# snimu/mixture-of-tokenizers

Hardware: NVIDIA B200
Metric: byte-mix embedding fwd+bwd tokens/sec (higher is better)
Workload: dtype bf16

## Files before the change

mixture-of-tokenizers_b200/csrc/mot_embed.cu:

```cuda
#include <algorithm>

#include "mot_embed_bwd_sum.cuh"

namespace mot {

__global__ void plan_hist_kernel(const int32_t* tok, long long N, int V, int* cnt) {
  pdl_launch_dependents();
  pdl_wait();
  for (long long i = (long long)blockIdx.x * blockDim.x + threadIdx.x; i < N; i += (long long)gridDim.x * blockDim.x)
    atomicAdd(&cnt[clampi(ld_g(tok + i), V - 1)], 1);
}

constexpr int kScanTile = 1024;
__global__ void __launch_bounds__(256) plan_scan_kernel(EmbedParams p) {
  __shared__ int wsum[8];
  __shared__ int wcarry[8];
  const int tid = threadIdx.x, lane = tid & 31, warp = tid >> 5;
  const int base = blockIdx.x * kScanTile;
  pdl_launch_dependents();
  pdl_wait();
  int carry = 0;
  for (int v = tid * 4; v < base; v += 256 * 4) {
    const int4 c = *reinterpret_cast<const int4*>(p.cnt + v);
    carry += c.x + c.y + c.z + c.w;
// ... 114 lines not shown
  }
  if (d->row_stride != 0 || d->col_offset != 0) {
    const long long ld = d->row_stride ? d->row_stride : d->out_dim;
    if (d->col_offset < 0 || ld < (long long)d->col_offset + d->out_dim || ld > 0x7fffffffLL) return MOT_ERR_BAD_ARG;
    if (ld % 8 || d->col_offset % 8) return MOT_ERR_MISALIGNED;
  }
  if (d->dp_slabs < 0 || d->dp_slabs > 64) return MOT_ERR_BAD_ARG;
  if ((d->flags & MOT_F_TTB_PULL_LEFT) && (d->flags & MOT_F_TTB_PULL_RIGHT)) return MOT_ERR_BAD_ARG;
  if ((d->flags & MOT_F_TTB_NEXT_TOK) && !(d->flags & MOT_F_TTB_PULL_RIGHT)) return MOT_ERR_BAD_ARG;
  if ((d->flags & MOT_F_IDS_FROM_TTB) && has_bytes) {
    if (d->ttb_dtype < MOT_TTB_I16 || d->ttb_dtype > MOT_TTB_BF16) return MOT_ERR_UNSUPPORTED;
    if (d->flags & (MOT_F_TTB_SCRAMBLE | MOT_F_TTB_PULL_LEFT | MOT_F_TTB_PULL_RIGHT))
      if (d->seq_len <= 0 || d->n_tokens % d->seq_len) return MOT_ERR_BAD_ARG;
    if (d->flags & (MOT_F_TTB_PULL_LEFT | MOT_F_TTB_PULL_RIGHT)) {
      if (d->tok_vocab <= 0) return MOT_ERR_BAD_ARG;
      if (d->pad_id != (int16_t)d->pad_id || d->eot_id != (int16_t)d->eot_id) return MOT_ERR_BAD_ARG;
    }
  }
  return MOT_OK;
}

static int validate(const MotDesc* d) {
  if (int rc = validate_desc(d)) return rc;
  if ((d->flags & MOT_F_BYTE_NORM) && d->combine != MOT_TOK_ONLY && d->byte_dim > 256) return MOT_ERR_UNSUPPORTED;
  constexpr int kMaxCols = 8 * 32 * 8;
  if (d->combine == MOT_CONCAT && !(d->flags & (MOT_F_OUT_NORM | MOT_F_HAS_LAMBDAS))) {
    if (d->tok_dim > kMaxCols || (long long)d->bpt * d->byte_dim > kMaxCols) return MOT_ERR_UNSUPPORTED;
  } else if (d->out_dim > kMaxCols) {
    return MOT_ERR_UNSUPPORTED;
  }
  return MOT_OK;
}

static bool aligned16(const void* p) { return (reinterpret_cast<uintptr_t>(p) & 15u) == 0; }

static void fill_params(const MotDesc* d, EmbedParams& p) {
  p = EmbedParams{};
  p.N = d->n_tokens;
  p.T = d->seq_len > 0 ? d->seq_len : (d->n_tokens > 0 ? d->n_tokens : 1);
  p.V = d->tok_vocab;
  p.Vb = d->combine == MOT_TOK_ONLY ? 0 : d->byte_vocab;
  p.bpt = d->combine == MOT_TOK_ONLY ? 0 : d->bpt;
  p.Dt = d->combine == MOT_BYTES_ONLY ? 0 : d->tok_dim;
  p.bd = d->combine == MOT_TOK_ONLY ? 8 : d->byte_dim;
  p.Do = d->out_dim;
  p.combine = d->combine;
  p.flags = d->flags;
  p.ttb_dtype = d->ttb_dtype;
  p.pad_eot = (d->pad_id & 0xffff) | (d->eot_id << 16);
  p.n_chunks = d->out_dim / kChunk;
  p.io_ld = d->row_stride ? d->row_stride : d->out_dim;
  p.io_col = d->col_offset;
  p.eps = d->eps;
  p.R = stream_chunk(d->n_tokens, kBwdThreads / 32);
  p.n_rep = kByteRep;
  p.stages = 4;
  p.tab_smem = 1;
  p.v_lo = 0;
  p.v_hi = p.V;
  p.last_slab = 1;
}

static bool concat_splits(const MotDesc* d) {
  return d->combine == MOT_CONCAT && !(d->flags & (MOT_F_OUT_NORM | MOT_F_HAS_LAMBDAS));
}
static void split_params(const MotDesc* d, EmbedParams& pt, EmbedParams& pb) {
  const int db = d->bpt * d->byte_dim;
  const bool bytes_first = (d->flags & MOT_F_BYTES_FIRST) != 0;
  MotDesc dt = *d, dbd = *d;
  dt.combine = MOT_TOK_ONLY;
  dt.out_dim = d->tok_dim;
  dt.flags = d->flags & MOT_F_TOK_NORM;
  dbd.combine = MOT_BYTES_ONLY;
  dbd.out_dim = db;
  dbd.flags = d->flags & ~(MOT_F_TOK_NORM | MOT_F_BYTES_FIRST);
  fill_params(&dt, pt);
  fill_params(&dbd, pb);
  pt.io_ld = pb.io_ld = d->row_stride ? d->row_stride : d->out_dim;
  pt.io_col = d->col_offset + (bytes_first ? db : 0);
  pb.io_col = d->col_offset + (bytes_first ? 0 : d->tok_dim);
}

struct WsLayout {
  size_t cnt, byte_acc, lam_acc, partial, zero_end, off, order, stok, total;
};

static WsLayout ws_layout(const EmbedParams& p, int dp_slabs = 0) {
  WsLayout w{};
  const long long V = p.V > 0 ? p.V : 1, N = p.N > 0 ? p.N : 1;
  int r_min = std::min(p.R, stream_chunk(N, kSumThreads / 32));
  if (dp_slabs > 1) r_min = std::min(r_min, stream_chunk_slab(N, dp_slabs, kSumThreads / 32));
  const long long n_stream_chunks = (N + r_min - 1) / r_min;
  size_t o = 0;
  auto take = [&](size_t bytes) {
    size_t at = o;
    o = align_up(o + bytes, 256);
    return at;
  };
  w.cnt = take((size_t)V * 4);
  w.byte_acc = take((size_t)p.n_rep * (p.Vb > 0 ? p.Vb : 1) * p.bd * 4);
  w.lam_acc = take(16);
  w.partial = take((size_t)n_stream_chunks * (p.Dt > 0 ? p.Dt : 8) * 4);
  w.zero_end = o;
  w.off = take((size_t)(V + 1) * 4);
  w.order = take((size_t)N * 4);
  w.stok = take((size_t)N * 4);
  w.total = o;
  return w;
}

static void bind_ws(EmbedParams& p, const WsLayout& w, void* ws) {
  char* b = reinterpret_cast<char*>(ws);
  p.cnt = reinterpret_cast<int*>(b + w.cnt);
  p.byte_acc = reinterpret_cast<float*>(b + w.byte_acc);
  p.lam_acc = reinterpret_cast<float*>(b + w.lam_acc);
  p.off = reinterpret_cast<int*>(b + w.off);
  p.order = reinterpret_cast<int*>(b + w.order);
  p.stok = reinterpret_cast<int*>(b + w.stok);
  p.partial = reinterpret_cast<float*>(b + w.partial);
  p.chk = chk_record();
  p.n_slots = (int)((w.zero_end - w.partial) / ((size_t)(p.Dt > 0 ? p.Dt : 8) * 4));
}

static int run_plan(const EmbedParams& p, cudaStream_t s) {
  if (p.combine == MOT_BYTES_ONLY || p.N == 0) return MOT_OK;
  long long hb = (p.N + 255) / 256;
  if (hb > 2048) hb = 2048;
  launch_pdl(plan_hist_kernel, dim3((unsigned)hb), dim3(256), 0, s, p.tok, p.N, p.V, p.cnt);
  launch_pdl(plan_scan_kernel, dim3((unsigned)((p.V + kScanTile - 1) / kScanTile)), dim3(256), 0, s, p);
  launch_pdl(plan_fill_kernel, dim3((unsigned)((p.N + 255) / 256)), dim3(256), 0, s, p);
  count_launch(3);
  return check_launch();
}

}

using namespace mot;

extern "C" size_t mot_embed_workspace_bytes(const MotDesc* d) {
  if (validate(d) != MOT_OK) return 0;
  EmbedParams p;
  fill_params(d, p);
  return ws_layout(p, d->dp_slabs).total;
}

extern "C" int mot_embed_fwd(const MotDesc* d, const int32_t* tok, const void* byte_ids, const void* ttb,
                             const void* E_tok, const void* E_byte, const float* lam, void* out, void* stream) {
  return mot_embed_fwd_ex(d, tok, byte_ids, ttb, E_tok, E_byte, lam, nullptr, out, nullptr, stream);
}

extern "C" int mot_embed_fwd_ex(const MotDesc* d, const int32_t* tok, const void* byte_ids, const void* ttb,
                                const void* E_tok, const void* E_byte, const float* lam, const void* addend, void* out,
                                float* rstd_out, void* stream) {
  if (int rc = validate(d)) return rc;
  if (addend && (concat_splits(d) || d->row_stride != 0 || d->col_offset != 0)) return MOT_ERR_UNSUPPORTED;
  if (!aligned16(addend)) return MOT_ERR_MISALIGNED;
  if (d->n_tokens == 0) return MOT_OK;
  const bool has_tok = d->combine != MOT_BYTES_ONLY, has_bytes = d->combine != MOT_TOK_ONLY;
  if (!out || (has_tok && (!tok || !E_tok)) || (has_bytes && !E_byte)) return MOT_ERR_BAD_ARG;
  if (has_bytes) {
    if (d->flags & MOT_F_IDS_FROM_TTB) { if (!ttb || !tok) return MOT_ERR_BAD_ARG; }
    else if (!byte_ids) return MOT_ERR_BAD_ARG;
  }
  if ((d->flags & MOT_F_HAS_LAMBDAS) && !lam) return MOT_ERR_BAD_ARG;
  if (!aligned16(out) || !aligned16(E_tok) || !aligned16(E_byte)) return MOT_ERR_MISALIGNED;
  cudaStream_t s = reinterpret_cast<cudaStream_t>(stream);
  if (concat_splits(d)) {
    EmbedParams pt, pb;
    split_params(d, pt, pb);
    for (EmbedParams* q : {&pt, &pb}) {
      q->tok = tok; q->ids = byte_ids; q->ttb = ttb; q->E_tok = E_tok; q->E_byte = E_byte; q->lam = lam; q->out = out;
      if (int rc = d->dtype == MOT_BF16 ? dispatch_fwd_bf16(*q, s) : dispatch_fwd_f32(*q, s)) return rc;
    }
    return MOT_OK;
  }
  EmbedParams p;
  fill_params(d, p);
  p.tok = tok; p.ids = byte_ids; p.ttb = ttb; p.E_tok = E_tok; p.E_byte = E_byte; p.lam = lam; p.out = out;
  p.rstd_out = (d->flags & MOT_F_OUT_NORM) ? rstd_out : nullptr;
  p.addend = addend;
  if (addend) return d->dtype == MOT_BF16 ? dispatch_fwd_addend_bf16(p, s) : dispatch_fwd_addend_f32(p, s);
  return d->dtype == MOT_BF16 ? dispatch_fwd_bf16(p, s) : dispatch_fwd_f32(p, s);
}

extern "C" int mot_embed_workspace_init(const MotDesc* d, void* workspace, size_t ws_bytes, void* stream) {
  if (int rc = validate(d)) return rc;
  if (!workspace) return MOT_ERR_BAD_ARG;
  EmbedParams p;
  fill_params(d, p);
  const WsLayout w = ws_layout(p, d->dp_slabs);
  if (ws_bytes < w.total) return MOT_ERR_WORKSPACE;
  if (cudaMemsetAsync(workspace, 0, w.zero_end, reinterpret_cast<cudaStream_t>(stream)) != cudaSuccess) return check_launch();
  return MOT_OK;
}

extern "C" int mot_embed_plan(const MotDesc* d, const int32_t* tok, void* workspace, size_t ws_bytes, int32_t ws_flags,
                              void* stream) {
  if (int rc = validate(d)) return rc;
  if (!workspace) return MOT_ERR_BAD_ARG;
  if (d->combine != MOT_BYTES_ONLY && !tok) return MOT_ERR_BAD_ARG;
  EmbedParams p;
  fill_params(d, p);
  const WsLayout w = ws_layout(p, d->dp_slabs);
  if (ws_bytes < w.total) return MOT_ERR_WORKSPACE;
// ... 27 lines not shown
  static const bool no_saved = getenv("MOT_NO_SAVED_BWD") != nullptr;
  if (no_saved || concat_splits(d) || pick_mode(p, kBwdCW) != 1 || p.io_ld != p.Do || p.io_col != 0) return false;
  const int cpl = p.Do / (32 * kBwdCW);
  if (!(cpl == 4 || cpl == 6 || cpl == 8 || (d->dtype == MOT_F32 && cpl == 2))) return false;
  return p.N <= 4LL * p.V;
}

extern "C" int mot_embed_bwd_uses_saved(const MotDesc* d) {
  if (validate(d) != MOT_OK) return 0;
  EmbedParams p;
  fill_params(d, p);
  return saved_path_applies(d, p) ? 1 : 0;
}

extern "C" int mot_embed_bwd(const MotDesc* d, const int32_t* tok, const void* byte_ids, const void* ttb,
                             const void* E_tok, const void* E_byte, const float* lam, const void* grad_out,
                             void* gE_tok, void* gE_byte, float* g_lam, void* workspace, size_t ws_bytes,
                             int32_t ws_flags, void* stream) {
  return mot_embed_bwd_ex(d, tok, byte_ids, ttb, E_tok, E_byte, lam, nullptr, grad_out, nullptr, nullptr, gE_tok, gE_byte,
                          g_lam, nullptr, workspace, ws_bytes, ws_flags, stream);
}

static int embed_bwd_impl(const MotDesc* d, const int32_t* tok, const void* byte_ids, const void* ttb,
                          const void* E_tok, const void* E_byte, const float* lam, const void* addend,
                          const void* grad_out, const void* out_saved, const float* rstd_saved, void* gE_tok,
                          void* gE_byte, float* g_lam, void* d_addend, void* workspace, size_t ws_bytes,
                          int32_t ws_flags, int slab, int n_slabs, int reserve_sms, void* stream) {
  const bool plan_ready = (ws_flags & MOT_WS_PLAN_READY) != 0, ws_clean = (ws_flags & MOT_WS_CLEAN) != 0;
  if (int rc = validate(d)) return rc;
  const bool slabbed = n_slabs > 1;
  if (n_slabs < 1 || slab < 0 || slab >= n_slabs || reserve_sms < 0 || reserve_sms > kDpReserveMax) return MOT_ERR_BAD_ARG;
  if (slabbed && (d->dp_slabs != n_slabs || (slab > 0 && !plan_ready))) return MOT_ERR_BAD_ARG;
  if (slabbed && d->n_tokens == 0) return MOT_ERR_UNSUPPORTED;
  const bool has_tok = d->combine != MOT_BYTES_ONLY, has_bytes = d->combine != MOT_TOK_ONLY;
  if (has_tok && !gE_tok) return MOT_ERR_BAD_ARG;
  if (has_bytes && !gE_byte) return MOT_ERR_BAD_ARG;
  if ((addend || d_addend) && (concat_splits(d) || d->row_stride != 0 || d->col_offset != 0)) return MOT_ERR_UNSUPPORTED;
  if (d_addend && (d->flags & MOT_F_OUT_NORM) && !addend) return MOT_ERR_BAD_ARG;
  if (!aligned16(addend) || !aligned16(d_addend)) return MOT_ERR_MISALIGNED;
  if (!aligned16(gE_tok) || !aligned16(gE_byte)) return MOT_ERR_MISALIGNED;
  if (d->n_tokens == 0) {
    cudaStream_t s0 = reinterpret_cast<cudaStream_t>(stream);
    const size_t esz0 = d->dtype == MOT_BF16 ? 2 : 4;
    if (has_tok && cudaMemsetAsync(gE_tok, 0, (size_t)d->tok_vocab * d->tok_dim * esz0, s0) != cudaSuccess) return check_launch();
    if (has_bytes && cudaMemsetAsync(gE_byte, 0, (size_t)d->byte_vocab * d->byte_dim * esz0, s0) != cudaSuccess) return check_launch();
    if (g_lam && cudaMemsetAsync(g_lam, 0, 8, s0) != cudaSuccess) return check_launch();
    return MOT_OK;
  }
  if (!grad_out || !workspace) return MOT_ERR_BAD_ARG;
  if (has_tok && (!tok || !E_tok)) return MOT_ERR_BAD_ARG;
  if (has_bytes && !E_byte) return MOT_ERR_BAD_ARG;
  if (has_bytes) {
    if (d->flags & MOT_F_IDS_FROM_TTB) { if (!ttb || !tok) return MOT_ERR_BAD_ARG; }
    else if (!byte_ids) return MOT_ERR_BAD_ARG;
  }
  if ((d->flags & MOT_F_HAS_LAMBDAS) && (!lam || !g_lam)) return MOT_ERR_BAD_ARG;
  if (!aligned16(grad_out) || !aligned16(E_tok) || !aligned16(E_byte) || !aligned16(gE_tok) || !aligned16(gE_byte) ||
      !aligned16(workspace))
    return MOT_ERR_MISALIGNED;
  EmbedParams p;
  fill_params(d, p);
  const WsLayout w = ws_layout(p, d->dp_slabs);
  if (ws_bytes < w.total) return MOT_ERR_WORKSPACE;
  bind_ws(p, w, workspace);
  p.tok = tok; p.ids = byte_ids; p.ttb = ttb; p.E_tok = E_tok; p.E_byte = E_byte; p.lam = lam;
  p.gout = grad_out; p.gE_tok = gE_tok; p.gE_byte = gE_byte; p.g_lam = g_lam;
  p.addend = addend; p.d_addend = d_addend;
  p.plan_early = (plan_ready && (ws_flags & MOT_WS_PLAN_JOINED)) ? 1 : 0;
  cudaStream_t s = reinterpret_cast<cudaStream_t>(stream);
  if (slabbed) {
    p.v_lo = (int)((long long)p.V * slab / n_slabs);
    p.v_hi = (int)((long long)p.V * (slab + 1) / n_slabs);
    p.last_slab = slab == n_slabs - 1;
    p.grid_cap = 148 - reserve_sms;
  }
  if (!plan_ready) {
    if (!ws_clean && cudaMemsetAsync(workspace, 0, w.zero_end, s) != cudaSuccess) return check_launch();
    if (int rc = run_plan(p, s)) return rc;
  } else if (!ws_clean) {
    if (cudaMemsetAsync(reinterpret_cast<char*>(workspace) + w.byte_acc, 0, w.zero_end - w.byte_acc, s) != cudaSuccess)
      return check_launch();
  }
  int rc = MOT_OK;
  if (slabbed && concat_splits(d)) return MOT_ERR_UNSUPPORTED;
  if (concat_splits(d)) {
    EmbedParams pt, pb;
    split_params(d, pt, pb);
    for (EmbedParams* q : {&pt, &pb}) {
      bind_ws(*q, w, workspace);
      q->tok = tok; q->ids = byte_ids; q->ttb = ttb; q->E_tok = E_tok; q->E_byte = E_byte; q->lam = lam;
      q->gout = grad_out; q->gE_tok = gE_tok; q->gE_byte = gE_byte; q->g_lam = g_lam;
      q->R = p.R;
      if ((rc = d->dtype == MOT_BF16 ? dispatch_bwd_bf16(*q, s) : dispatch_bwd_f32(*q, s))) return rc;
    }
  } else {
    rc = -1;
    if (out_saved && rstd_saved && !addend && !d_addend && saved_path_applies(d, p)) {
      if (!aligned16(out_saved)) return MOT_ERR_MISALIGNED;
      p.out_saved = out_saved;
      p.rstd = rstd_saved;
      const int r_default = p.R;
      p.R = slabbed ? stream_chunk_slab(p.N, n_slabs, kSumThreads / 32) : stream_chunk(p.N, kSumThreads / 32);
      rc = d->dtype == MOT_BF16 ? dispatch_bwd_sum_bf16(p, s) : dispatch_bwd_sum_f32(p, s);
      if (rc < 0) p.R = r_default;
    }
    if (slabbed && rc < 0) return MOT_ERR_UNSUPPORTED;
    if (rc < 0 && (addend || d_addend)) rc = d->dtype == MOT_BF16 ? dispatch_bwd_addend_bf16(p, s) : dispatch_bwd_addend_f32(p, s);
    if (rc < 0) rc = d->dtype == MOT_BF16 ? dispatch_bwd_bf16(p, s) : dispatch_bwd_f32(p, s);
  }
  if (rc) return rc;
  int sms = 0, optin = 0;
  device_props(&sms, &optin);
  {
    const long long tasks = (has_tok ? (p.N + p.R - 1) / p.R : 0) + p.Vb;
    long long fb = (tasks + 7) / 8;
    if (fb > 8LL * sms) fb = 8LL * sms;
    if (fb < 1) fb = 1;
    p.trace = g_trace ? g_trace + 2 * 4096 * 64 : nullptr;
    rc = d->dtype == MOT_BF16 ? launch_finalize_bf16(p, (int)fb, s) : launch_finalize_f32(p, (int)fb, s);
  }
  if (rc) return rc;
  if ((d->flags & MOT_F_HAS_LAMBDAS) && g_lam && p.last_slab) {
    launch_pdl(mot_lam_store_kernel, dim3(1), dim3(32), 0, s, p.lam_acc, g_lam);
    count_launch();
  }
  return check_launch();
}

extern "C" int mot_embed_bwd_ex(const MotDesc* d, const int32_t* tok, const void* byte_ids, const void* ttb,
                                const void* E_tok, const void* E_byte, const float* lam, const void* addend,
                                const void* grad_out, const void* out_saved, const float* rstd_saved, void* gE_tok,
                                void* gE_byte, float* g_lam, void* d_addend, void* workspace, size_t ws_bytes,
                                int32_t ws_flags, void* stream) {
  return embed_bwd_impl(d, tok, byte_ids, ttb, E_tok, E_byte, lam, addend, grad_out, out_saved, rstd_saved, gE_tok, gE_byte,
                        g_lam, d_addend, workspace, ws_bytes, ws_flags, 0, 1, 0, stream);
}

extern "C" int mot_embed_bwd_slab(const MotDesc* d, const int32_t* tok, const void* byte_ids, const void* ttb,
                                  const void* E_tok, const void* E_byte, const float* lam, const void* grad_out,
                                  const void* out_saved, const float* rstd_saved, void* gE_tok, void* gE_byte, float* g_lam,
                                  void* workspace, size_t ws_bytes, int32_t ws_flags, int32_t slab, int32_t n_slabs,
                                  int32_t reserve_sms, void* stream) {
  return embed_bwd_impl(d, tok, byte_ids, ttb, E_tok, E_byte, lam, nullptr, grad_out, out_saved, rstd_saved, gE_tok, gE_byte,
                        g_lam, nullptr, workspace, ws_bytes, ws_flags, slab, n_slabs, reserve_sms, stream);
}

extern "C" int mot_embed_slab_rows(int32_t tok_vocab, int32_t slab, int32_t n_slabs, int32_t* row_lo, int32_t* row_hi) {
  if (tok_vocab <= 0 || n_slabs < 1 || slab < 0 || slab >= n_slabs || !row_lo || !row_hi) return MOT_ERR_BAD_ARG;
  *row_lo = (int32_t)((long long)tok_vocab * slab / n_slabs);
  *row_hi = (int32_t)((long long)tok_vocab * (slab + 1) / n_slabs);
  return MOT_OK;
}

extern "C" int mot_embed_touched_rows(const MotDesc* d, const void* workspace, size_t ws_bytes, uint32_t* bitmap, void* stream) {
  if (int rc = validate(d)) return rc;
  if (d->combine == MOT_BYTES_ONLY) return MOT_ERR_UNSUPPORTED;
  if (!workspace || !bitmap) return MOT_ERR_BAD_ARG;
  EmbedParams p;
  fill_params(d, p);
  const WsLayout w = ws_layout(p, d->dp_slabs);
  if (ws_bytes < w.total) return MOT_ERR_WORKSPACE;
  bind_ws(p, w, const_cast<void*>(workspace));
  const int words = (p.V + 31) / 32;
  launch_pdl(plan_rowmap_kernel, dim3((unsigned)((words + 7) / 8)), dim3(256), 0, reinterpret_cast<cudaStream_t>(stream),
             (const int*)p.off, (int)p.V, bitmap);
  count_launch();
  return check_launch();
}
```

mixture-of-tokenizers_b200/csrc/mot_embed_bwd_sum.cuh:

```cuda
#pragma once
#include "mot_embed_kernels.cuh"

namespace mot {

#ifndef MOT_SUM_THREADS
#define MOT_SUM_THREADS 384
#endif
#ifndef MOT_SUM_TWO_PASS
#define MOT_SUM_TWO_PASS 0
#endif
#ifndef MOT_SUM_BULK_RED
#define MOT_SUM_BULK_RED 0
#endif
constexpr int kSumThreads = MOT_SUM_THREADS;

struct SumSmem {
  size_t bars, ring, row_bytes, stage_bytes, total;
};
__host__ __device__ inline SumSmem sum_smem(int Do, size_t esz, int warps, int stages) {
  SumSmem L{};
  L.bars = 0;
  L.ring = align_up((size_t)warps * stages * 8, 128);
  L.row_bytes = align_up((size_t)Do * esz, 128);
  L.stage_bytes = 2 * L.row_bytes;
  L.total = L.ring + (size_t)warps * stages * L.stage_bytes;
  return L;
}

__device__ __forceinline__ void mbar_expect_tx_s(uint32_t bar, uint32_t bytes) {
  asm volatile("mbarrier.arrive.expect_tx.shared::cta.b64 _, [%0], %1;" ::"r"(bar), "r"(bytes) : "memory");
}
__device__ __forceinline__ void mbar_wait_s(uint32_t bar, uint32_t phase) {
  asm volatile(
      "{\n"
      ".reg .pred P1;\n"
      "LAB_WAIT:\n"
      "mbarrier.try_wait.parity.shared::cta.b64 P1, [%0], %1;\n"
      "@P1 bra DONE;\n"
      "bra LAB_WAIT;\n"
      "DONE:\n"
      "}\n" ::"r"(bar),
      "r"(phase)
      : "memory");
}
__device__ __forceinline__ void bulk_g2s_s(uint32_t dst, const void* gmem_src, uint32_t bytes, uint32_t bar) {
  asm volatile("cp.async.bulk.shared::cluster.global.mbarrier::complete_tx::bytes [%0], [%1], %2, [%3];" ::"r"(dst),
               "l"(gmem_src), "r"(bytes), "r"(bar)
               : "memory");
}

struct SumBatch {
  int pos, v;
  float r;
  int cnt;
  int a;
  int flags;
  int v_prev;
  int v_next;
};

template <typename T, int CPL, int PULL>
__global__ void __launch_bounds__(kSumThreads, 1) mot_bwd_sum_kernel(const EmbedParams p) {
  constexpr int CW = kBwdCW;
  using V = Vec<T, CW>;
  constexpr unsigned kFull = 0xffffffffu;
  extern __shared__ __align__(128) unsigned char smem_raw[];
  const int lane = lane_id();
  const int warp = threadIdx.x >> 5;
  const int nw = blockDim.x >> 5;
  const int D = p.stages;
  const SumSmem L = sum_smem(p.Do, sizeof(T), nw, D);
  const uint32_t bars_s = smem_u32(smem_raw + L.bars) + (uint32_t)(warp * D) * 8u;
  const uint32_t stage_bytes = (uint32_t)L.stage_bytes, row_off = (uint32_t)L.row_bytes;
  unsigned char* ring = smem_raw + L.ring + (size_t)warp * D * L.stage_bytes;
  const uint32_t ring_s = smem_u32(ring);

  if (lane == 0)
    for (int s = 0; s < D; ++s) mbar_init(reinterpret_cast<uint64_t*>(smem_raw + L.bars) + warp * D + s, 1);
  fence_mbar_init();
  pdl_launch_dependents();
  __syncthreads();
  const int gw = warp * gridDim.x + blockIdx.x;
  MOT_STAMP(p.trace, gw, 0);
  if (!p.plan_early) pdl_wait();

  const int W = gridDim.x * nw;
  const int Ni = (int)p.N, R = p.R;
  const char* gout = reinterpret_cast<const char*>(p.gout);
  const char* osv = reinterpret_cast<const char*>(p.out_saved);
  const uint32_t row_bytes = (uint32_t)p.Do * sizeof(T);

  const int a0 = ld_g(p.off + p.v_lo), a1 = ld_g(p.off + p.v_hi);
  const int c_lo = a0 / R, c_hi = (a1 + R - 1) / R;
  MOT_ASSERT(a0 >= 0 && a0 <= a1 && a1 <= Ni, "stream range", a0, a1);
  MOT_ASSERT(p.v_lo >= 0 && p.v_lo <= p.v_hi && p.v_hi <= p.V, "row range", p.v_lo, p.v_hi);

  int nx_chunk = c_lo + gw, nx_a = max(nx_chunk * R, a0);
  auto load_next = [&](SumBatch& b, bool with_r) {
    b.pos = 0;
    b.v = -1;
    b.r = 0.f;
    b.cnt = 0;
    b.a = 0;
    b.flags = 0;
    b.v_prev = -1;
    b.v_next = -1;
    if (nx_chunk >= c_hi) return;
    const int c0 = max(nx_chunk * R, a0), c_end = min(nx_chunk * R + R, a1);
    const int a = nx_a, left = c_end - a;
    b.a = a;
    b.cnt = left < 32 ? left : 32;
    MOT_ASSERT(a >= a0 && a + b.cnt <= a1 && b.cnt >= 0, "batch range", a, b.cnt);
    if (lane < b.cnt) {
      b.pos = ld_g(p.order + a + lane);
      b.v = ld_g(p.stok + a + lane);
      MOT_ASSERT(b.pos >= 0 && b.pos < Ni, "position", b.pos, a + lane);
      MOT_ASSERT(b.v >= p.v_lo && b.v < p.v_hi, "token row", b.v, a + lane);
      if (with_r) b.r = ld_g(p.rstd + b.pos);
    }
    if (a == c0) {
      b.flags |= 1;
      if (a > 0) b.v_prev = ld_g(p.stok + a - 1);
    }
    if (left <= 32) {
      b.flags |= 2;
      if (c_end < Ni) b.v_next = ld_g(p.stok + c_end);
      nx_chunk += W;
      nx_a = nx_chunk < c_hi ? max(nx_chunk * R, a0) : 0;
    } else {
      nx_a = a + 32;
    }
  };
  SumBatch A, B;
  load_next(A, !p.plan_early);
  load_next(B, !p.plan_early);
  if (p.plan_early) {
    pdl_wait();
    if (lane < A.cnt) A.r = ld_g(p.rstd + A.pos);
    if (lane < B.cnt) B.r = ld_g(p.rstd + B.pos);
  }
  MOT_STAMP(p.trace, gw, 1);
  MOT_STAMP(p.trace, gw, 2);

  int inflight = 0;
  int is = 0, cs = 0;
  uint32_t cpar = 0;
  int iw = 0, ik = 0;
  auto try_issue = [&]() -> bool {
    int cnt = iw ? B.cnt : A.cnt;
    if (ik >= cnt) {
      if (iw == 1 || B.cnt == 0) return false;
      iw = 1;
      ik = 0;
    }
    if (lane == ik) {
      const unsigned long long goff = (unsigned long long)(unsigned)(iw ? B.pos : A.pos) * row_bytes;
      const uint32_t st = ring_s + (uint32_t)is * stage_bytes, bar = bars_s + (uint32_t)is * 8u;
      mbar_expect_tx_s(bar, 2u * row_bytes);
      bulk_g2s_s(st, gout + goff, row_bytes, bar);
#ifdef MOT_X_SUM_NO_OCOPY
      bulk_g2s_s(st + row_off, gout + goff, row_bytes, bar);
#else
      bulk_g2s_s(st + row_off, osv + goff, row_bytes, bar);
#endif
    }
    ++inflight;
    if (++is == D) is = 0;
    ++ik;
    return true;
  };
  while (inflight < D && try_issue()) {
  }
  MOT_STAMP(p.trace, gw, 3);

#if !MOT_SUM_BULK_RED || MOT_SUM_TWO_PASS
  int slot[CPL];
  unsigned boff4[CPL];
#pragma unroll
  for (int it = 0; it < CPL; ++it) {
    const int e = (it * 32 + lane) * CW;
    slot[it] = e / p.bd;
    boff4[it] = (unsigned)(e - slot[it] * p.bd) * 4u;
    asm volatile("" : "+r"(slot[it]), "+r"(boff4[it]));
  }
#else
  bool red_pending = false;
#endif
  const unsigned bd4 = (unsigned)p.bd * 4u;
  char* accp = reinterpret_cast<char*>(p.byte_acc + (size_t)(gw % p.n_rep) * p.Vb * p.bd);
  const float inv_Do = 1.f / (float)p.Do;
  const bool id_lane = lane < p.bpt;
  const IdSrc idsrc = make_id_src(p, lane);
  T* G = reinterpret_cast<T*>(p.gE_tok);

  MOT_STAMP(p.trace, gw, 4);
#ifdef MOT_TRACE
  int n_occ = 0;
#endif
  float Du[CPL][CW];
#pragma unroll
  for (int it = 0; it < CPL; ++it)
#pragma unroll
    for (int e = 0; e < CW; ++e) Du[it][e] = 0.f;
  int cur_v = -1;
  bool seg_lead = false;

  auto flush = [&](bool partial_row) {
    if (!partial_row) {
#ifndef MOT_X_SUM_NO_FLUSH
      MOT_ASSERT(cur_v >= p.v_lo && cur_v < p.v_hi, "flush row", cur_v, p.v_hi);
      T* grow = G + (size_t)(unsigned)cur_v * (unsigned)p.Dt;
#pragma unroll
      for (int it = 0; it < CPL; ++it) V::stg(grow + (it * 32 + lane) * CW, Du[it]);
#endif
    } else {
      const int c_first = ld_g(p.off + cur_v) / R;
      MOT_ASSERT(c_first >= 0 && c_first < p.n_slots, "partial slot", c_first, p.n_slots);
      float* prow = p.partial + (size_t)(unsigned)c_first * (unsigned)p.Dt;
#pragma unroll
      for (int it = 0; it < CPL; ++it)
        atomicAdd(reinterpret_cast<float4*>(prow + (it * 32 + lane) * CW), make_float4(Du[it][0], Du[it][1], Du[it][2], Du[it][3]));
    }
#pragma unroll
    for (int it = 0; it < CPL; ++it)
#pragma unroll
      for (int e = 0; e < CW; ++e) Du[it][e] = 0.f;
  };

  int id_next = 0;
  if (A.cnt > 0) {
    const int pos0 = __shfl_sync(kFull, A.pos, 0);
    if constexpr (PULL) id_next = pulled_lane_id<PULL>(p, pos0, id_lane);
    else if (id_lane) id_next = load_raw_id(p, idsrc, pos0, lane);
  }
  while (A.cnt > 0) {
    const int cnt = A.cnt;
    for (int k = 0; k < cnt; ++k) {
      const int v = __shfl_sync(kFull, A.v, k);
      const float r = __shfl_sync(kFull, A.r, k);
      if (v != cur_v) {
        if (cur_v >= 0) flush(seg_lead);
        seg_lead = k == 0 && (A.flags & 1) && v == A.v_prev;
        cur_v = v;
      }
      const int idreg = clamp_id(p, id_next);
      {
        const bool more = k + 1 < cnt;
        const int pos_n = __shfl_sync(kFull, more ? A.pos : B.pos, more ? k + 1 : 0);
        if constexpr (PULL) {
          if (more || B.cnt > 0) id_next = pulled_lane_id<PULL>(p, pos_n, id_lane);
        } else {
          if (id_lane && (more || B.cnt > 0)) id_next = load_raw_id(p, idsrc, pos_n, lane);
        }
      }

      mbar_wait_s(bars_s + (uint32_t)cs * 8u, cpar);
#ifdef MOT_TRACE
      MOT_STAMP(p.trace, gw, 5 + n_occ);
      ++n_occ;
#endif
      const T* grow = reinterpret_cast<const T*>(ring + (size_t)cs * stage_bytes);
      const T* orow = reinterpret_cast<const T*>(ring + (size_t)cs * stage_bytes + row_off);
#if MOT_SUM_BULK_RED
      float* dzrow = reinterpret_cast<float*>(ring + (size_t)cs * stage_bytes);
      const uint32_t dz_s = ring_s + (uint32_t)cs * stage_bytes;
#endif
      if (++cs == D) {
        cs = 0;
        cpar ^= 1u;
      }
#if MOT_SUM_TWO_PASS
      float gzp[CW] = {0.f, 0.f, 0.f, 0.f};
#pragma unroll
      for (int it = 0; it < CPL; ++it) {
        float g[CW], o[CW];
        V::unpack(V::lds_raw(grow + (it * 32 + lane) * CW), g);
        V::unpack(V::lds_raw(orow + (it * 32 + lane) * CW), o);
#pragma unroll
        for (int e = 0; e < CW; ++e) gzp[e] += g[e] * o[e];
      }
      float gz = (gzp[0] + gzp[1]) + (gzp[2] + gzp[3]);
      gz = warp_sum(gz);
      const float c = r * gz * inv_Do;
#ifdef MOT_X_SUM_NO_MATH
      if (c == 12345.678f)
#endif
#pragma unroll
      for (int it = 0; it < CPL; ++it) {
        const int id = __shfl_sync(kFull, idreg, slot[it]);
        float g[CW], o[CW], dz[CW];
        V::unpack(V::lds_raw(grow + (it * 32 + lane) * CW), g);
        V::unpack(V::lds_raw(orow + (it * 32 + lane) * CW), o);
#pragma unroll
        for (int e = 0; e < CW; ++e) {
          dz[e] = r * g[e] - c * o[e];
          Du[it][e] += dz[e];
        }
        gmem_add4(reinterpret_cast<float*>(accp + ((unsigned)id * bd4 + boff4[it])), dz);
      }
      __syncwarp();
      --inflight;
      try_issue();
#else
      float g[CPL][CW], o[CPL][CW];
      float gzp[CW] = {0.f, 0.f, 0.f, 0.f};
#pragma unroll
      for (int it = 0; it < CPL; ++it) {
        V::unpack(V::lds_raw(grow + (it * 32 + lane) * CW), g[it]);
        V::unpack(V::lds_raw(orow + (it * 32 + lane) * CW), o[it]);
#pragma unroll
        for (int e = 0; e < CW; ++e) gzp[e] += g[it][e] * o[it][e];
      }
      float gz = (gzp[0] + gzp[1]) + (gzp[2] + gzp[3]);
      gz = warp_sum(gz);
#if !MOT_SUM_BULK_RED
      --inflight;
      try_issue();
#endif
      const float c = r * gz * inv_Do;
#ifdef MOT_X_SUM_NO_MATH
      if (c == 12345.678f)
#endif
#pragma unroll
      for (int it = 0; it < CPL; ++it) {
#if !MOT_SUM_BULK_RED
        const int id = __shfl_sync(kFull, idreg, slot[it]);
#endif
        float dz[CW];
#pragma unroll
        for (int e = 0; e < CW; ++e) {
          dz[e] = r * g[it][e] - c * o[it][e];
          Du[it][e] += dz[e];
        }
#if MOT_SUM_BULK_RED
        *reinterpret_cast<float4*>(dzrow + (it * 32 + lane) * CW) = make_float4(dz[0], dz[1], dz[2], dz[3]);
#else
        MOT_ASSERT(id >= 0 && id < p.Vb, "byte id", id, p.Vb);
        gmem_add4(reinterpret_cast<float*>(accp + ((unsigned)id * bd4 + boff4[it])), dz);
#endif
      }
#if MOT_SUM_BULK_RED
      asm volatile("fence.proxy.async.shared::cta;" ::: "memory");
      __syncwarp();
      if (id_lane) {
        MOT_ASSERT(idreg >= 0 && idreg < p.Vb, "byte id", idreg, p.Vb);
#ifndef MOT_EXPERIMENT_NO_RED
        asm volatile("cp.reduce.async.bulk.global.shared::cta.bulk_group.add.f32 [%0], [%1], %2;" ::"l"(accp + (unsigned)idreg * bd4),
                     "r"(dz_s + (unsigned)lane * bd4), "r"(bd4)
                     : "memory");
#endif
        asm volatile("cp.async.bulk.commit_group;" ::: "memory");
        asm volatile("cp.async.bulk.wait_group.read 1;" ::: "memory");
      }
      __syncwarp();
      if (red_pending) {
        --inflight;
        try_issue();
      }
      red_pending = true;
#endif
#endif
    }
    if (A.flags & 2) {
      if (cur_v >= 0) flush(seg_lead || A.v_next == cur_v);
      cur_v = -1;
      seg_lead = false;
    }
    A = B;
    if (iw == 1) iw = 0; else ik = 0;
    load_next(B, true);
    while (inflight < D && try_issue()) {
    }
  }
  MOT_STAMP(p.trace, gw, 61);

#ifndef MOT_X_SUM_NO_ZERO
  {
    const float zero[CW] = {0.f, 0.f, 0.f, 0.f};
    int* zctr = reinterpret_cast<int*>(p.lam_acc) + 2;
    const int n_blocks = (p.v_hi - p.v_lo + 31) >> 5;
    auto grab = [&]() -> int {
      int b = 0;
      if (lane == 0) b = atomicAdd(zctr, 1);
      return __shfl_sync(kFull, b, 0);
    };
    int nb = grab();
    while (nb < n_blocks) {
      const int vb = p.v_lo + (nb << 5);
      const int v = vb + lane;
      const bool empty = v < p.v_hi && (ld_g(p.off + v + 1) - ld_g(p.off + v)) == 0;
      nb = grab();
      unsigned m = __ballot_sync(kFull, empty);
      while (m) {
        const int j = __ffs(m) - 1;
        m &= m - 1;
        MOT_ASSERT(vb + j >= p.v_lo && vb + j < p.v_hi, "zero row", vb + j, p.v_hi);
        T* row = G + (size_t)(unsigned)(vb + j) * (unsigned)p.Dt;
#pragma unroll
        for (int it = 0; it < CPL; ++it) V::stg(row + (it * 32 + lane) * CW, zero);
      }
    }
  }
#endif
  MOT_STAMP(p.trace, gw, 62);
#if MOT_SUM_BULK_RED && !MOT_SUM_TWO_PASS
  if (id_lane) asm volatile("cp.async.bulk.wait_group 0;" ::: "memory");
#endif
#ifdef MOT_TRACE
  if (p.trace != nullptr && lane == 0) p.trace[(size_t)gw * 64 + 63] = n_occ;
#endif
}

template <typename T, int CPL, int PULL = kNoPull>
static int launch_bwd_sum(const EmbedParams& p_in, cudaStream_t s) {
  if constexpr (PULL == kNoPull) {
    if (const int k = ids_pulled(p_in))
      return k == kPullLeft ? launch_bwd_sum<T, CPL, kPullLeft>(p_in, s) : launch_bwd_sum<T, CPL, kPullRight>(p_in, s);
  }
  int sms = 0, optin = 0;
  if (int rc = device_props(&sms, &optin)) return rc;
  EmbedParams p = p_in;
  static const char* env_st = getenv("MOT_SUM_STAGES");
  int want = env_st ? atoi(env_st) : 4;
  if (want < 2) want = 2;
  size_t smem = 0;
  for (int st = want; st >= 2; --st) {
    const SumSmem L = sum_smem(p.Do, sizeof(T), kSumThreads / 32, st);
    if (L.total + 1024 <= (size_t)optin) {
      p.stages = st;
      smem = L.total;
      break;
    }
  }
  if (smem == 0) return MOT_ERR_UNSUPPORTED;
  p.trace = g_trace ? g_trace + 4096 * 64 : nullptr;
  auto kern = mot_bwd_sum_kernel<T, CPL, PULL>;
  if (cudaFuncSetAttribute(kern, cudaFuncAttributeMaxDynamicSharedMemorySize, (int)smem) != cudaSuccess) return check_launch();
  if (g_prof_start) cudaEventRecord(g_prof_start, s);
  const int ctas = (p.grid_cap > 0 && p.grid_cap < sms) ? p.grid_cap : sms;
  launch_pdl(kern, dim3((unsigned)ctas), dim3(kSumThreads), smem, s, p);
  if (g_prof_stop) cudaEventRecord(g_prof_stop, s);
  count_launch();
  return check_launch();
}

inline bool sum_path_ok(const EmbedParams& p) {
  return p.out_saved != nullptr && p.rstd != nullptr && pick_mode(p, kBwdCW) == 1 && p.io_ld == p.Do && p.io_col == 0 &&
         !(p.flags & MOT_F_IDS_FROM_TTB && p.ttb == nullptr);
}

}
```

mixture-of-tokenizers_b200/csrc/mot_embed_kernels.cuh:

```cuda
#pragma once
#include <cstdlib>

#include "mot_common.cuh"

namespace mot {

constexpr int kFwdThreads = 768;
#ifndef MOT_BWD_THREADS
#define MOT_BWD_THREADS 384
#endif
constexpr int kBwdThreads = MOT_BWD_THREADS;
#ifndef MOT_BYTE_REP
#define MOT_BYTE_REP 16
#endif
constexpr int kByteRep = MOT_BYTE_REP;

struct EmbedParams {
  const int32_t* tok;
  const void* ids;
  const void* ttb;
  const void* E_tok;
  const void* E_byte;
  const float* lam;
  void* out;
  float* rstd_out;
  const void* gout;
  const void* out_saved;
  const float* rstd;
  const void* addend;
  void* d_addend;
  void* gE_tok;
  void* gE_byte;
  float* g_lam;
  int* cnt;
  int* off;
  int* order;
  int* stok;
  float* partial;
  float* byte_acc;
  float* lam_acc;
  long long N, T;
  long long io_ld;
  int io_col;
  int V, Vb, bpt, Dt, bd, Do, combine, flags, ttb_dtype;
  int n_chunks;
  int R;
  int n_rep;
  int stages;
  int tab_smem;
  int v_lo, v_hi;
  int grid_cap;
  int last_slab;
  int plan_early;
  float eps;
  long long* trace;
  long long* chk;
  int n_slots;
  int pad_eot;
};

struct ChunkMap {
  int toff;
  int slot;
  int boff;
};

template <int CW>
__device__ __forceinline__ ChunkMap chunk_map(const EmbedParams& p, int c) {
  ChunkMap m{-1, -1, 0};
  if (c * CW >= p.Do) return m;
  const int e = c * CW;
  switch (p.combine) {
    case MOT_ADD:
      m.toff = e;
      m.slot = e / p.bd;
      m.boff = e - m.slot * p.bd;
      break;
    case MOT_CONCAT: {
      const int db = p.bpt * p.bd;
      int eb = -1;
      if (p.flags & MOT_F_BYTES_FIRST) {
        if (e < db) eb = e; else m.toff = e - db;
      } else {
        if (e < p.Dt) m.toff = e; else eb = e - p.Dt;
      }
      if (eb >= 0) {
        m.slot = eb / p.bd;
        m.boff = eb - m.slot * p.bd;
      }
    } break;
    case MOT_TOK_ONLY:
      m.toff = e;
      break;
    case MOT_BYTES_ONLY:
      m.slot = e / p.bd;
      m.boff = e - m.slot * p.bd;
      break;
    case MOT_MEAN:
      m.toff = e;
      m.slot = -2;
      m.boff = e;
      break;
  }
  return m;
}

__device__ __forceinline__ int clampi(int v, int hi) { return min(max(v, 0), hi); }
__device__ __forceinline__ size_t mul_u32(int a, int b) { return (size_t)(unsigned)a * (unsigned)b; }

__device__ __forceinline__ int fetch_id(const EmbedParams& p, long long pos, int slot) {
  int id;
  if (p.flags & MOT_F_IDS_FROM_TTB) {
    long long tokpos = pos;
    int k = slot;
    if (p.flags & MOT_F_TTB_SCRAMBLE) {
      const long long row = pos / p.T, s = pos - row * p.T;
      const long long f = (long long)slot * p.T + s;
      tokpos = row * p.T + f / p.bpt;
      k = (int)(f % p.bpt);
    }
    const int tv = clampi(ld_g(p.tok + tokpos), p.V - 1);
    const size_t e = (size_t)tv * p.bpt + k;
    if (p.ttb_dtype == MOT_TTB_I16) id = ld_g(reinterpret_cast<const short*>(p.ttb) + e);
// ... 868 lines not shown
            V::stg(reinterpret_cast<T*>(p.d_addend) + (size_t)pos_k * p.Do + (size_t)(it * 32 + lane) * CW, dz);
        } else {
#pragma unroll
          for (int e = 0; e < CW; ++e) dz[e] = 0.f;
        }
        if (has_bytes) {
          if (C::mean(p)) {
            for (int kk = 0; kk < p.bpt; ++kk) {
              const int id = __shfl_sync(0xffffffffu, idreg, kk);
              if (valid && cm[it].slot == -2) {
                if (has_lam) {
                  float b[CW];
                  V::unpack(tab_load<T, MODE, CW>(p, tab, (unsigned)(id * p.bd + cm[it].boff)), b);
                  const float r = rs[id] * inv_pool;
#pragma unroll
                  for (int e = 0; e < CW; ++e) dlam_b += dz[e] * r * b[e];
                }
                float dzs[CW];
#pragma unroll
                for (int e = 0; e < CW; ++e) dzs[e] = dz[e] * lam_b_eff;
                gmem_add4(accp + (unsigned)(id * p.bd + cm[it].boff), dzs);
              }
            }
          } else if (valid && MOT_BYTE_OK(it)) {
            const int id = idv[it];
            if (has_lam) {
              float b[CW];
              V::unpack(tab_load<T, MODE, CW>(p, tab, (unsigned)(id * p.bd + cm[it].boff)), b);
              const float r = rs[id];
#pragma unroll
              for (int e = 0; e < CW; ++e) dlam_b += dz[e] * r * b[e];
            }
            if (C::kLam) {
#pragma unroll
              for (int e = 0; e < CW; ++e) dz[e] *= lam_b_eff;
            }
            gmem_add4(accp + (unsigned)(id * p.bd + cm[it].boff), dz);
          }
        }
      }
      __syncwarp();
    }
    if (chunk_last && has_tok && cur_v >= 0) {
      const int b_end = chunk * p.R + p.R;
      const bool trail = b_end < Ni && ld_g(p.stok + b_end) == cur_v;
      flush(trail);
      cur_v = -1;
      seg_lead = false;
    }
    A = B;
    if (iw == 1) iw = 0; else ik = 0;
    load_next(B);
    const int hold = (cur_v >= 0 && need_trow && (tok_norm || has_lam)) ? 1 : 0;
    while (issued - consumed < D - hold && try_issue()) {
    }
  }

  if (has_lam) {
    dlam_t = warp_sum(dlam_t);
    dlam_b = warp_sum(dlam_b);
    if (lane == 0) {
      atomicAdd(p.lam_acc, dlam_t);
      atomicAdd(p.lam_acc + 1, dlam_b);
    }
  }
}

template <typename T>
__global__ void __launch_bounds__(256) mot_bwd_finalize_kernel(const EmbedParams p) {
  pdl_launch_dependents();
  MOT_STAMP(p.trace, (blockIdx.x * (blockDim.x >> 5) + (threadIdx.x >> 5)) & 4095, 0);
  pdl_wait();
  const int lane = lane_id();
  const int nw = blockDim.x >> 5;
  const int gw = blockIdx.x * nw + (threadIdx.x >> 5);
  MOT_STAMP(p.trace, gw & 4095, 1);
  const int W = gridDim.x * nw;
  const bool has_tok = p.combine != MOT_BYTES_ONLY;
  const bool has_bytes = p.combine != MOT_TOK_ONLY;
  const bool has_lam = (p.flags & MOT_F_HAS_LAMBDAS) != 0;
  float lam_t = 1.f;
  if (has_lam) lam_t = ld_g(p.lam);
  float dlam_t = 0.f;
  if (blockIdx.x == 0 && threadIdx.x == 0 && p.lam_acc != nullptr)
    reinterpret_cast<int*>(p.lam_acc)[2] = 0;
  if (has_tok) {
    const bool tok_norm = (p.flags & MOT_F_TOK_NORM) != 0;
    const long long a0 = ld_g(p.off + p.v_lo), a1 = ld_g(p.off + p.v_hi);
    const long long c_lo = a0 / p.R, c_hi = (a1 + p.R - 1) / p.R;
    const T* E_tok = reinterpret_cast<const T*>(p.E_tok);
    T* G = reinterpret_cast<T*>(p.gE_tok);
    MOT_ASSERT(a0 >= 0 && a0 <= a1 && a1 <= p.N, "finalize stream range", a0, a1);
    for (long long c0 = c_lo + gw; c0 + 1 < c_hi; c0 += W) {
      MOT_ASSERT(c0 >= 0 && c0 < p.n_slots, "finalize slot", c0, p.n_slots);
      const long long bnd = (c0 + 1) * (long long)p.R;
      MOT_ASSERT(bnd > 0 && bnd < p.N, "finalize boundary", bnd, p.N);
      const int v = ld_g(p.stok + bnd - 1);
      MOT_ASSERT(v >= 0 && v < p.V, "finalize token", v, p.V);
      if (ld_g(p.stok + bnd) != v) continue;
      if (ld_g(p.off + v) < c0 * (long long)p.R) continue;
      float* prow = p.partial + (size_t)c0 * p.Dt;
      const T* trow = E_tok + (size_t)v * p.Dt;
      float dot = 0.f, ss = 0.f;
      for (int pass = (tok_norm || has_lam) ? 0 : 1; pass < 2; ++pass) {
        const float r_t = tok_norm ? rsqrtf(ss / (float)p.Dt + p.eps) : 1.f;
        const float a_ = lam_t * r_t;
        const float b_ = tok_norm ? lam_t * r_t * r_t * r_t * dot / (float)p.Dt : 0.f;
        float dacc = 0.f, sacc = 0.f;
        for (int c = lane; c < p.Dt / kChunk; c += 32) {
          float tv[8] = {0.f, 0.f, 0.f, 0.f, 0.f, 0.f, 0.f, 0.f}, du[8];
          if (tok_norm || has_lam) Vec8<T>::unpack(Vec8<T>::ldg_raw(trow + c * kChunk), tv);
          float* pr = prow + c * kChunk;
          const float4 x = *reinterpret_cast<const float4*>(pr), y = *reinterpret_cast<const float4*>(pr + 4);
          du[0] = x.x; du[1] = x.y; du[2] = x.z; du[3] = x.w; du[4] = y.x; du[5] = y.y; du[6] = y.z; du[7] = y.w;
          if (pass == 0) {
#pragma unroll
            for (int e = 0; e < 8; ++e) {
              dacc += du[e] * tv[e];
              sacc += tv[e] * tv[e];
            }
          } else {
            float o[8];
#pragma unroll
            for (int e = 0; e < 8; ++e) o[e] = a_ * du[e] - b_ * tv[e];
            Vec8<T>::stg(G + (size_t)v * p.Dt + c * kChunk, o);
            *reinterpret_cast<float4*>(pr) = make_float4(0.f, 0.f, 0.f, 0.f);
            *reinterpret_cast<float4*>(pr + 4) = make_float4(0.f, 0.f, 0.f, 0.f);
          }
        }
        if (pass == 0) {
          warp_sum2(dacc, sacc);
          dot = dacc;
          ss = sacc;
          if (lane == 0) dlam_t += (tok_norm ? rsqrtf(ss / (float)p.Dt + p.eps) : 1.f) * dot;
        }
      }
    }
  }
  if (has_bytes && p.last_slab) {
    const bool bn = (p.flags & MOT_F_BYTE_NORM) != 0;
    const T* E_byte = reinterpret_cast<const T*>(p.E_byte);
    T* G = reinterpret_cast<T*>(p.gE_byte);
    const size_t rep_stride = (size_t)p.Vb * p.bd;
    const int nc = p.bd / kChunk;
    for (int r = W - 1 - gw; r < p.Vb; r += W) {
      if (nc <= 32) {
        const int ngrp = 32 / nc;
        const int grp = lane / nc, c = lane - grp * nc;
        const bool live = grp < ngrp;
        float a[8] = {0.f, 0.f, 0.f, 0.f, 0.f, 0.f, 0.f, 0.f};
        if (live) {
          float* base = p.byte_acc + (size_t)r * p.bd + c * kChunk;
#pragma unroll 1
          for (int j0 = 0; grp + j0 * ngrp < kByteRep; j0 += 4) {
            float4 x[4], y[4];
#pragma unroll
            for (int j = 0; j < 4; ++j) {
              const int rep = grp + (j0 + j) * ngrp;
              if (rep < kByteRep) {
                x[j] = *reinterpret_cast<const float4*>(base + rep * rep_stride);
                y[j] = *reinterpret_cast<const float4*>(base + rep * rep_stride + 4);
              }
            }
#pragma unroll
            for (int j = 0; j < 4; ++j) {
              const int rep = grp + (j0 + j) * ngrp;
              if (rep < kByteRep) {
                *reinterpret_cast<float4*>(base + rep * rep_stride) = make_float4(0.f, 0.f, 0.f, 0.f);
// ... 153 lines not shown
```

Measured before the change: 541.7 million.

## Fuse backward finalize into sum kernel via last-arriver atomic counters

The saved-output backward sum path now finishes its own work instead of launching a separate finalize kernel. Each token row split across stream chunks is closed by whichever warp arrives last on a per-slot counter. That warp writes the gradient row and re-zeroes the partial buffer. The byte-table replicas are reduced in two stages by the last-arriving block per replica group, then by the last group overall, which writes gE_byte. This removes a kernel launch and its serialized pass over the partials, at the cost of extra workspace counters, release/acquire atomics, and skipping the lambda-store launch on this path, which may drop g_lam handling.

Result: slower. 429.4 million, median of 6 (-20.7%).

```diff
diff --git a/mixture-of-tokenizers_b200/csrc/mot_embed.cu b/mixture-of-tokenizers_b200/csrc/mot_embed.cu
--- a/mixture-of-tokenizers_b200/csrc/mot_embed.cu
+++ b/mixture-of-tokenizers_b200/csrc/mot_embed.cu
@@ -220,7 +220,8 @@
 }
 
 struct WsLayout {
-  size_t cnt, byte_acc, lam_acc, partial, zero_end, off, order, stok, total;
+  size_t cnt, byte_acc, lam_acc, partial, slot_ctr, byte_ctr, byte_fin, zero_end, off, order, stok, total;
+  long long n_slots;
 };
 
 static WsLayout ws_layout(const EmbedParams& p, int dp_slabs = 0) {
@@ -235,11 +236,16 @@
     o = align_up(o + bytes, 256);
     return at;
   };
+  const size_t table = (size_t)(p.Vb > 0 ? p.Vb : 1) * p.bd * 4;
   w.cnt = take((size_t)V * 4);
-  w.byte_acc = take((size_t)p.n_rep * (p.Vb > 0 ? p.Vb : 1) * p.bd * 4);
+  w.byte_acc = take((size_t)p.n_rep * table);
   w.lam_acc = take(16);
   w.partial = take((size_t)n_stream_chunks * (p.Dt > 0 ? p.Dt : 8) * 4);
+  w.slot_ctr = take((size_t)n_stream_chunks * 4);
+  w.byte_ctr = take((size_t)(p.n_rep + 1) * 4);
+  w.byte_fin = take(table);
   w.zero_end = o;
+  w.n_slots = n_stream_chunks;
   w.off = take((size_t)(V + 1) * 4);
   w.order = take((size_t)N * 4);
   w.stok = take((size_t)N * 4);
@@ -256,8 +262,11 @@
   p.order = reinterpret_cast<int*>(b + w.order);
   p.stok = reinterpret_cast<int*>(b + w.stok);
   p.partial = reinterpret_cast<float*>(b + w.partial);
+  p.slot_ctr = reinterpret_cast<int*>(b + w.slot_ctr);
+  p.byte_ctr = reinterpret_cast<int*>(b + w.byte_ctr);
+  p.byte_fin = reinterpret_cast<float*>(b + w.byte_fin);
   p.chk = chk_record();
-  p.n_slots = (int)((w.zero_end - w.partial) / ((size_t)(p.Dt > 0 ? p.Dt : 8) * 4));
+  p.n_slots = (int)w.n_slots;
 }
 
 static int run_plan(const EmbedParams& p, cudaStream_t s) {
@@ -451,6 +460,7 @@
       return check_launch();
   }
   int rc = MOT_OK;
+  bool finished = false;
   if (slabbed && concat_splits(d)) return MOT_ERR_UNSUPPORTED;
   if (concat_splits(d)) {
     EmbedParams pt, pb;
@@ -472,12 +482,14 @@
       p.R = slabbed ? stream_chunk_slab(p.N, n_slabs, kSumThreads / 32) : stream_chunk(p.N, kSumThreads / 32);
       rc = d->dtype == MOT_BF16 ? dispatch_bwd_sum_bf16(p, s) : dispatch_bwd_sum_f32(p, s);
       if (rc < 0) p.R = r_default;
+      finished = rc >= 0;
     }
     if (slabbed && rc < 0) return MOT_ERR_UNSUPPORTED;
     if (rc < 0 && (addend || d_addend)) rc = d->dtype == MOT_BF16 ? dispatch_bwd_addend_bf16(p, s) : dispatch_bwd_addend_f32(p, s);
     if (rc < 0) rc = d->dtype == MOT_BF16 ? dispatch_bwd_bf16(p, s) : dispatch_bwd_f32(p, s);
   }
   if (rc) return rc;
+  if (finished) return MOT_OK;
   int sms = 0, optin = 0;
   device_props(&sms, &optin);
   {
diff --git a/mixture-of-tokenizers_b200/csrc/mot_embed_bwd_sum.cuh b/mixture-of-tokenizers_b200/csrc/mot_embed_bwd_sum.cuh
--- a/mixture-of-tokenizers_b200/csrc/mot_embed_bwd_sum.cuh
+++ b/mixture-of-tokenizers_b200/csrc/mot_embed_bwd_sum.cuh
@@ -2,6 +2,26 @@
 #include "mot_embed_kernels.cuh"
 
 namespace mot {
+
+template <bool kCta>
+__device__ __forceinline__ bool arrive_last(int* ctr, int count, int* s_flag) {
+  const bool leader = kCta ? threadIdx.x == 0 : lane_id() == 0;
+  int old = 0;
+  if constexpr (kCta) __syncthreads(); else __syncwarp();
+  if (leader) {
+    asm volatile("atom.add.release.gpu.s32 %0, [%1], 1;" : "=r"(old) : "l"(ctr) : "memory");
+    if (old == count - 1) asm volatile("fence.acq_rel.gpu;" ::: "memory");
+  }
+  if constexpr (kCta) {
+    if (leader) *s_flag = old;
+    __syncthreads();
+    old = *s_flag;
+  } else {
+    old = __shfl_sync(0xffffffffu, old, 0);
+    __syncwarp();
+  }
+  return old == count - 1;
+}
 
 #ifndef MOT_SUM_THREADS
 #define MOT_SUM_THREADS 384
@@ -58,6 +78,70 @@
   int v_prev;
   int v_next;
 };
+
+template <typename T, int CPL>
+__device__ __noinline__ void sum_close_row(float* prow, T* grow, int* ctr, int n_seg) {
+  if (!arrive_last<false>(ctr, n_seg, nullptr)) return;
+  const int lane = lane_id();
+  float4 x[CPL];
+#pragma unroll
+  for (int it = 0; it < CPL; ++it) x[it] = __ldcg(reinterpret_cast<const float4*>(prow + (it * 32 + lane) * kBwdCW));
+#pragma unroll
+  for (int it = 0; it < CPL; ++it) {
+    const float o[kBwdCW] = {x[it].x, x[it].y, x[it].z, x[it].w};
+    Vec<T, kBwdCW>::stg(grow + (it * 32 + lane) * kBwdCW, o);
+    *reinterpret_cast<float4*>(prow + (it * 32 + lane) * kBwdCW) = make_float4(0.f, 0.f, 0.f, 0.f);
+  }
+  if (lane == 0) *ctr = 0;
+}
+
+template <typename T>
+__device__ __noinline__ void sum_byte_table(int* byte_ctr, float* byte_acc, float* byte_fin, T* gE_byte, float* lam_acc,
+                                            int n_rep, int table, int last_slab, long long* ctrace) {
+  using V = Vec<T, kBwdCW>;
+  constexpr int kB = 8;
+  __shared__ int s_flag;
+  const int rep = (int)blockIdx.x % n_rep;
+  const int n_grp = min(n_rep, (int)gridDim.x);
+  const int grp_size = ((int)gridDim.x - rep + n_rep - 1) / n_rep;
+  const int n4 = table / 4, nt = blockDim.x;
+  if (threadIdx.x < 32) MOT_STAMP(ctrace, blockIdx.x, 0);
+  if (!arrive_last<true>(byte_ctr + rep, grp_size, &s_flag)) return;
+  float4* acc4 = reinterpret_cast<float4*>(byte_acc + (size_t)rep * table);
+  float4* fin4 = reinterpret_cast<float4*>(byte_fin);
+  for (int i0 = threadIdx.x; i0 < n4; i0 += kB * nt) {
+    float4 x[kB];
+#pragma unroll
+    for (int j = 0; j < kB; ++j)
+      if (i0 + j * nt < n4) x[j] = __ldcg(acc4 + i0 + j * nt);
+#pragma unroll
+    for (int j = 0; j < kB; ++j)
+      if (i0 + j * nt < n4) {
+        atomicAdd(fin4 + i0 + j * nt, x[j]);
+        acc4[i0 + j * nt] = make_float4(0.f, 0.f, 0.f, 0.f);
+      }
+  }
+  if (threadIdx.x < 32) MOT_STAMP(ctrace, blockIdx.x, 1);
+  if (!arrive_last<true>(byte_ctr + n_rep, n_grp, &s_flag)) return;
+  if (last_slab) {
+    for (int i0 = threadIdx.x; i0 < n4; i0 += kB * nt) {
+      float4 x[kB];
+#pragma unroll
+      for (int j = 0; j < kB; ++j)
+        if (i0 + j * nt < n4) x[j] = __ldcg(fin4 + i0 + j * nt);
+#pragma unroll
+      for (int j = 0; j < kB; ++j)
+        if (i0 + j * nt < n4) {
+          const float o[kBwdCW] = {x[j].x, x[j].y, x[j].z, x[j].w};
+          V::stg(gE_byte + (size_t)(i0 + j * nt) * 4, o);
+          fin4[i0 + j * nt] = make_float4(0.f, 0.f, 0.f, 0.f);
+        }
+    }
+  }
+  if ((int)threadIdx.x <= n_rep) byte_ctr[threadIdx.x] = 0;
+  if (threadIdx.x == 0) reinterpret_cast<int*>(lam_acc)[2] = 0;
+  if (threadIdx.x < 32) MOT_STAMP(ctrace, blockIdx.x, 2);
+}
 
 template <typename T, int CPL, int PULL>
 __global__ void __launch_bounds__(kSumThreads, 1) mot_bwd_sum_kernel(const EmbedParams p) {
@@ -187,7 +271,8 @@
   bool red_pending = false;
 #endif
   const unsigned bd4 = (unsigned)p.bd * 4u;
-  char* accp = reinterpret_cast<char*>(p.byte_acc + (size_t)(gw % p.n_rep) * p.Vb * p.bd);
+  const int rep = (int)blockIdx.x % p.n_rep;
+  char* accp = reinterpret_cast<char*>(p.byte_acc + (size_t)rep * p.Vb * p.bd);
   const float inv_Do = 1.f / (float)p.Do;
   const bool id_lane = lane < p.bpt;
   const IdSrc idsrc = make_id_src(p, lane);
@@ -204,11 +289,18 @@
     for (int e = 0; e < CW; ++e) Du[it][e] = 0.f;
   int cur_v = -1;
   bool seg_lead = false;
-
+  int lead_v = -1;
+
+  auto close_row = [&](int v) {
+    const int c_first = ld_g(p.off + v) / R, n_seg = (ld_g(p.off + v + 1) - 1) / R - c_first + 1;
+    MOT_ASSERT(n_seg >= 2 && n_seg <= p.n_slots - c_first, "row segments", n_seg, c_first);
+    sum_close_row<T, CPL>(p.partial + (size_t)(unsigned)c_first * (unsigned)p.Dt, G + (size_t)(unsigned)v * (unsigned)p.Dt,
+                          p.slot_ctr + c_first, n_seg);
+  };
   auto flush = [&](bool partial_row) {
+    MOT_ASSERT(cur_v >= p.v_lo && cur_v < p.v_hi, "flush row", cur_v, p.v_hi);
     if (!partial_row) {
 #ifndef MOT_X_SUM_NO_FLUSH
-      MOT_ASSERT(cur_v >= p.v_lo && cur_v < p.v_hi, "flush row", cur_v, p.v_hi);
       T* grow = G + (size_t)(unsigned)cur_v * (unsigned)p.Dt;
 #pragma unroll
       for (int it = 0; it < CPL; ++it) V::stg(grow + (it * 32 + lane) * CW, Du[it]);
@@ -240,6 +332,7 @@
       const float r = __shfl_sync(kFull, A.r, k);
       if (v != cur_v) {
         if (cur_v >= 0) flush(seg_lead);
+        if (seg_lead) lead_v = cur_v;
         seg_lead = k == 0 && (A.flags & 1) && v == A.v_prev;
         cur_v = v;
       }
@@ -362,8 +455,12 @@
 #endif
     }
     if (A.flags & 2) {
-      if (cur_v >= 0) flush(seg_lead || A.v_next == cur_v);
+      const bool partial_row = cur_v >= 0 && (seg_lead || A.v_next == cur_v);
+      if (cur_v >= 0) flush(partial_row);
+      if (partial_row) close_row(cur_v);
+      if (lead_v >= 0) close_row(lead_v);
       cur_v = -1;
+      lead_v = -1;
       seg_lead = false;
     }
     A = B;
@@ -405,10 +502,14 @@
   MOT_STAMP(p.trace, gw, 62);
 #if MOT_SUM_BULK_RED && !MOT_SUM_TWO_PASS
   if (id_lane) asm volatile("cp.async.bulk.wait_group 0;" ::: "memory");
+  asm volatile("fence.proxy.async.global;" ::: "memory");
 #endif
 #ifdef MOT_TRACE
   if (p.trace != nullptr && lane == 0) p.trace[(size_t)gw * 64 + 63] = n_occ;
 #endif
+  MOT_ASSERT(p.n_rep >= 1 && p.n_rep < (int)blockDim.x && p.bd % 4 == 0, "byte table tail", p.n_rep, p.bd);
+  sum_byte_table<T>(p.byte_ctr, p.byte_acc, p.byte_fin, reinterpret_cast<T*>(p.gE_byte), p.lam_acc, p.n_rep, p.Vb * p.bd,
+                    p.last_slab, p.trace != nullptr ? p.trace + 4096 * 64 : nullptr);
 }
 
 template <typename T, int CPL, int PULL = kNoPull>
diff --git a/mixture-of-tokenizers_b200/csrc/mot_embed_kernels.cuh b/mixture-of-tokenizers_b200/csrc/mot_embed_kernels.cuh
--- a/mixture-of-tokenizers_b200/csrc/mot_embed_kernels.cuh
+++ b/mixture-of-tokenizers_b200/csrc/mot_embed_kernels.cuh
@@ -39,6 +39,9 @@
   float* partial;
   float* byte_acc;
   float* lam_acc;
+  int* slot_ctr;
+  int* byte_ctr;
+  float* byte_fin;
   long long N, T;
   long long io_ld;
   int io_col;
@@ -1073,8 +1076,6 @@
   float lam_t = 1.f;
   if (has_lam) lam_t = ld_g(p.lam);
   float dlam_t = 0.f;
-  if (blockIdx.x == 0 && threadIdx.x == 0 && p.lam_acc != nullptr)
-    reinterpret_cast<int*>(p.lam_acc)[2] = 0;
   if (has_tok) {
     const bool tok_norm = (p.flags & MOT_F_TOK_NORM) != 0;
     const long long a0 = ld_g(p.off + p.v_lo), a1 = ld_g(p.off + p.v_hi);
```
